# zxhuang1698/ZeroShape

Measured on AMD Instinct MI355X. Metric: sdf_query_points_per_sec_vox128, higher is better.
Workload: dtype f16x3

## Files before the change

### zeroshape_amd/csrc/sdf_decoder_split.hip

```cpp
#include "zs_common.h"
#include <stdlib.h>
#include "sdf_layout.h"
#include "sdf_math.h"
#include "zs_split16.h"
#include "sdf_query.h"
#include "../../include/zeroshape_hip.h"

#include <math.h>
#include <stdint.h>
#include <type_traits>

namespace {

using namespace zs::lay;
using namespace zs::qry;
using zs::dm::gelu_erf;
using zs::dm::softplus100;

typedef float f32x16 __attribute__((ext_vector_type(16)));
typedef float f32x4 __attribute__((ext_vector_type(4)));
typedef float f32x2 __attribute__((ext_vector_type(2)));
typedef unsigned u32x4 __attribute__((ext_vector_type(4)));

constexpr float S_GUARD = 64.0f;
constexpr int KB_U4 = 128;
constexpr int CK = 8;
constexpr int KPW = CK / WAVES;
constexpr int CHUNK_BYTES = CK * KB_U4 * 16;
constexpr int NBUF = 2;
constexpr int KB_TOTAL = G_TOTAL / 2;
constexpr int PRM_WINDOW = 4096;
constexpr int STAGE_FLOATS = NBUF * CHUNK_BYTES / 4;
constexpr int SLAB_TILES = NT - 1;
constexpr int SLAB_U4 = SLAB_TILES * 4 * 64;
constexpr int ZTILES_F4 = NT * 4 * 64;
static_assert(ZSLAB_F4 == 3 * ZTILES_F4, "the workspace slab holds three skip layers' feat partial products");
static_assert(B0_TABLE_FLOATS == PRM_WINDOW, "block0_window_kernel / block0_stream_kernel index an image's table by PRM_WINDOW");
constexpr int LDS_FLOATS = PRM_WINDOW + STAGE_FLOATS + WAVES * SLAB_U4 * 4;
static_assert(LDS_FLOATS * 4 == 160 * 1024, "the kernel owns the whole LDS of a CU");
static_assert(KB_TOTAL % CK == 0 && CK % WAVES == 0 && KPW * 2048 <= 4096, "chunking");
static_assert((RING * GROUP_FLOATS + PARAM_FLOATS) * 4 >= NBUF * CHUNK_BYTES, "prefetch stays inside the program");

constexpr int W_PP = P_PP;
constexpr int W_BLK = P_BLK0;
constexpr int W_IA = P_LNFG;
constexpr int W_IB = P_IMPL_PAIR + P_IMPL_PAIR_STRIDE;
static_assert(P_BLK_STRIDE <= PRM_WINDOW && W_IB - W_IA <= PRM_WINDOW && P_USED - W_IB <= PRM_WINDOW,
              "params windows");

#define DEV __device__ __forceinline__

DEV void pin(u32x4 &a, u32x4 &b) { asm volatile("" : "+v"(a), "+v"(b) : : "memory"); }

using zs::s16::mfma3;
using zs::s16::split2;

struct PT {
    u32x4 v[4];
};
template <typename T>
DEV PT pack_tile(const T &x) {
    PT p;
#pragma unroll
    for (int j = 0; j < 2; j++)
#pragma unroll
        for (int i = 0; i < 4; i++) {
            unsigned h, l;
            split2(x[8 * j + 2 * i], x[8 * j + 2 * i + 1], h, l);
            p.v[2 * j][i] = h;
            p.v[2 * j + 1][i] = l;
        }
    return p;
}

DEV void glds_kblocks(const char *gsrc, unsigned lds_dst) {
#ifdef ZS_EXP_NO_DMA
    if (gsrc != nullptr) return;
#endif
    asm volatile("s_mov_b32 m0, %1\n\ts_nop 0\n\tglobal_load_lds_dwordx4 %0, off"
                 "\n\tglobal_load_lds_dwordx4 %0, off offset:1024"
                 "\n\tglobal_load_lds_dwordx4 %0, off offset:2048"
                 "\n\tglobal_load_lds_dwordx4 %0, off offset:3072"
                 :
                 : "v"(gsrc), "s"(lds_dst)
                 : "memory");
}

struct AStream {
    const u32x4 *buf[NBUF];
    unsigned dst[NBUF];
    u32x4 hi, lo;
    const char *gsrc;

    DEV void init(const char *prog, u32x4 *stage, unsigned stage_addr, int wave, int lane) {
        const char *g = prog + wave * (KPW * KB_U4 * 16) + lane * 16;
        asm volatile("s_waitcnt vmcnt(0) lgkmcnt(0)\n\ts_barrier" ::: "memory");
#pragma unroll
        for (int i = 0; i < NBUF; i++) {
            buf[i] = stage + i * (CK * KB_U4) + lane;
            dst[i] = stage_addr + i * CHUNK_BYTES + wave * (KPW * KB_U4 * 16);
            glds_kblocks(g + i * CHUNK_BYTES, dst[i]);
        }
        gsrc = g + NBUF * CHUNK_BYTES;
        asm volatile("s_waitcnt vmcnt(4)\n\ts_barrier" ::: "memory");
        hi = buf[0][0];
        lo = buf[0][64];
    }
    template <int EXTRA_VM = 0>
    DEV void step(int pos, u32x4 &ahi, u32x4 &alo) {
        ahi = hi;
        alo = lo;
        if (pos == CK - 1) {
            static_assert(EXTRA_VM == 0 || EXTRA_VM == 4, "wait-count variants");
            if (EXTRA_VM == 4)
                asm volatile("s_waitcnt vmcnt(4) lgkmcnt(0)\n\ts_barrier" ::: "memory");
            else
                asm volatile("s_waitcnt vmcnt(0) lgkmcnt(0)\n\ts_barrier" ::: "memory");
            glds_kblocks(gsrc, dst[0]);
            gsrc += CHUNK_BYTES;
            const u32x4 *t = buf[0];
            const unsigned u = dst[0];
            buf[0] = buf[1];
            dst[0] = dst[1];
            buf[1] = t;
            dst[1] = u;
            hi = buf[0][0];
            lo = buf[0][64];
        } else {
#ifndef ZS_EXP_NO_AREAD
            hi = buf[0][(pos + 1) * KB_U4];
            lo = buf[0][(pos + 1) * KB_U4 + 64];
#endif
        }
    }
    DEV void seek(const char *base, int wave, int lane) { gsrc = base + wave * (KPW * KB_U4 * 16) + lane * 16; }
    DEV void drain() { asm volatile("s_waitcnt vmcnt(0) lgkmcnt(0)" ::: "memory"); }
};

struct Slab {
    u32x4 *fl;
    PT t7;
    DEV void store(int tile, const PT &p) {
        if (tile == SLAB_TILES) {
            t7 = p;
        } else {
#pragma unroll
            for (int q = 0; q < 4; q++) fl[(tile * 4 + q) * 64] = p.v[q];
        }
    }
};

DEV f32x16 zero16() {
    f32x16 v;
#pragma unroll
    for (int r = 0; r < 16; r++) v[r] = 0.f;
    return v;
}

struct NoSide {
    DEV void operator()(int, int) const {}
};
template <typename SIDE>
DEV void mfma3_gaps(f32x16 &acc, const u32x4 &ahi, const u32x4 &alo, const u32x4 &bhi, const u32x4 &blo, int kb,
                    SIDE &side) {
    using zs::s16::as_h;
    if (std::is_same<SIDE, NoSide>::value) {
        mfma3(acc, ahi, alo, bhi, blo);
        return;
    }
    acc = __builtin_amdgcn_mfma_f32_32x32x16_f16(as_h(alo), as_h(bhi), acc, 0, 0, 0);
    side(kb, 0);
    acc = __builtin_amdgcn_mfma_f32_32x32x16_f16(as_h(ahi), as_h(blo), acc, 0, 0, 0);
    side(kb, 1);
    acc = __builtin_amdgcn_mfma_f32_32x32x16_f16(as_h(ahi), as_h(bhi), acc, 0, 0, 0);
    side(kb, 2);
}

struct TilePacker {
    PT p;
    float prev;
    DEV void feed(int kb, float v) {
        if (kb & 1) {
            unsigned h, l;
            split2(prev, v, h, l);
            p.v[2 * (kb >> 3)][(kb & 7) >> 1] = h;
            p.v[2 * (kb >> 3) + 1][(kb & 7) >> 1] = l;
        }
        prev = v;
    }
};

struct GeluStager {
    float x, u, q, t, e, p;
    DEV void s0(float v) {
        x = v;
        u = fabsf(v) * 0.70710678118654752440f;
        q = (u * u) * -1.44269504088896340736f;
    }
    DEV void s1() { t = __builtin_amdgcn_rcpf(fmaf(0.3275911f, u, 1.0f)); }
    DEV void s2() {
        e = __builtin_amdgcn_exp2f(q);
        p = fmaf(0.75052702f, t, -1.02753365f);
    }
    DEV void s3() {
        p = fmaf(p, t, 1.00509130f);
        p = fmaf(p, t, -0.20116957f);
        p = fmaf(p, t, 0.18019173f);
        p = p * t;
        u = u * p;
    }
    DEV float s4() const { return fmaf(-u, e, fmaxf(x, 0.0f)); }
    DEV float all(float v) {
        s0(v); s1(); s2(); s3();
        return s4();
    }
    DEV void stage(int st, float v, int idx, TilePacker &pk) {
        if (st == 0) s0(v);
        else if (st == 1) s1();
        else if (st == 2) s2();
        else if (st == 3) s3();
        else if (st == 4) pk.feed(idx, s4());
    }
};
struct SoftplusStager {
    float x, t;
    DEV void s0(float v) {
        x = v;
        t = __builtin_amdgcn_exp2f(fabsf(v) * -144.26950408889634074f);
    }
    DEV void s1() { t = __builtin_amdgcn_logf(1.0f + t); }
    DEV float s2() const { return fmaf(t, 0.0069314718055994530942f, fmaxf(x, 0.0f)); }
};

DEV float kblock_gelu(f32x16 &acc, const u32x4 &ahi, const u32x4 &alo, const u32x4 &bhi, const u32x4 &blo, float x) {
    float u, q, d, t, e, m, p;
    const float c0 = 0.70710678118654752440f, c1 = 0.3275911f, c2 = -1.02753365f;
    asm volatile(
#ifndef ZS_EXP_TWO_TERM
                 "v_mfma_f32_32x32x16_f16 %[acc], %[alo], %[bh], %[acc]\n\t"
#endif
                 "v_mul_f32_e64 %[u], |%[x]|, %[c0]\n\t"
                 "v_mul_f32_e32 %[q], %[u], %[u]\n\t"
                 "v_mul_f32_e32 %[q], 0xbfb8aa3b, %[q]\n\t"
                 "v_fma_f32 %[d], %[u], %[c1], 1.0\n\t"
                 "v_mfma_f32_32x32x16_f16 %[acc], %[ahi], %[bl], %[acc]\n\t"
                 "v_rcp_f32_e32 %[t], %[d]\n\t"
                 "v_exp_f32_e32 %[e], %[q]\n\t"
                 "v_max_f32_e32 %[m], 0, %[x]\n\t"
                 "v_mfma_f32_32x32x16_f16 %[acc], %[ahi], %[bh], %[acc]\n\t"
                 "v_fmamk_f32 %[p], %[t], 0x3f40228a, %[c2]\n\t"
                 "v_fmaak_f32 %[p], %[p], %[t], 0x3f80a6d5\n\t"
                 "v_fmaak_f32 %[p], %[p], %[t], 0xbe4dff65\n\t"
                 "v_fmaak_f32 %[p], %[p], %[t], 0x3e38842e\n\t"
                 "v_mul_f32_e64 %[p], %[t], -%[p]\n\t"
                 "v_mul_f32_e32 %[p], %[u], %[p]\n\t"
                 "v_fmac_f32_e32 %[m], %[p], %[e]"
                 : [acc] "+v"(acc), [u] "=&v"(u), [q] "=&v"(q), [d] "=&v"(d), [t] "=&v"(t), [e] "=&v"(e), [m] "=&v"(m),
                   [p] "=&v"(p)
                 : [alo] "v"(alo), [ahi] "v"(ahi), [bh] "v"(bhi), [bl] "v"(blo), [x] "v"(x), [c0] "s"(c0), [c1] "s"(c1),
                   [c2] "v"(c2));
    return m;
}
DEV float kblock_softplus(f32x16 &acc, const u32x4 &ahi, const u32x4 &alo, const u32x4 &bhi, const u32x4 &blo, float x) {
    float t, m;
    const float c0 = -144.26950408889634074f;
    asm volatile(
#ifndef ZS_EXP_TWO_TERM
                 "v_mfma_f32_32x32x16_f16 %[acc], %[alo], %[bh], %[acc]\n\t"
#endif
                 "v_mul_f32_e64 %[t], |%[x]|, %[c0]\n\t"
                 "v_exp_f32_e32 %[t], %[t]\n\t"
                 "v_mfma_f32_32x32x16_f16 %[acc], %[ahi], %[bl], %[acc]\n\t"
                 "v_max_f32_e32 %[m], 0, %[x]\n\t"
                 "v_add_f32_e32 %[t], 1.0, %[t]\n\t"
                 "v_log_f32_e32 %[t], %[t]\n\t"
                 "v_mfma_f32_32x32x16_f16 %[acc], %[ahi], %[bh], %[acc]\n\t"
                 "s_nop 0\n\t"
                 "v_fmac_f32_e32 %[m], 0x3be32166, %[t]"
                 : [acc] "+v"(acc), [t] "=&v"(t), [m] "=&v"(m)
                 : [alo] "v"(alo), [ahi] "v"(ahi), [bh] "v"(bhi), [bl] "v"(blo), [x] "v"(x), [c0] "s"(c0));
    return m;
}

DEV void mfma_settle(f32x16 &acc) { asm volatile("s_nop 7\n\ts_nop 3" : "+v"(acc)); }

template <int KT, int EXTRA_VM = 0, typename SIDE = NoSide>
DEV void gemm_reg(AStream &s, const PT *X, f32x16 &acc, SIDE side = SIDE()) {
#pragma unroll
    for (int kt = 0; kt < KT; kt++)
#pragma unroll
        for (int j = 0; j < 2; j++) {
            u32x4 ahi, alo;
            s.step((kt * 2 + j) & (CK - 1), ahi, alo);
            pin(ahi, alo);
            mfma3_gaps(acc, ahi, alo, X[kt].v[2 * j], X[kt].v[2 * j + 1], kt * 2 + j, side);
        }
}
template <typename SIDE>
DEV void mfma3_breg(f32x16 &acc, const u32x4 &ahi, const u32x4 &alo, const u32x4 &bhi, const u32x4 &blo, int kb,
                    SIDE &side) {
    asm volatile("s_nop 1\n\tv_mfma_f32_32x32x16_f16 %0, %1, %2, %0" : "+v"(acc) : "v"(alo), "a"(bhi));
    side(kb, 0);
    asm volatile("s_nop 1\n\tv_mfma_f32_32x32x16_f16 %0, %1, %2, %0" : "+v"(acc) : "v"(ahi), "a"(blo));
    side(kb, 1);
    asm volatile("s_nop 1\n\tv_mfma_f32_32x32x16_f16 %0, %1, %2, %0" : "+v"(acc) : "v"(ahi), "a"(bhi));
    side(kb, 2);
}
template <int KT, typename SIDE = NoSide>
DEV void gemm_areg(AStream &s, const PT *X, f32x16 &acc, SIDE side = SIDE()) {
#pragma unroll
    for (int kt = 0; kt < KT; kt++)
#pragma unroll
        for (int j = 0; j < 2; j++) {
            u32x4 ahi, alo;
            s.step((kt * 2 + j) & (CK - 1), ahi, alo);
            pin(ahi, alo);
            mfma3_breg(acc, ahi, alo, X[kt].v[2 * j], X[kt].v[2 * j + 1], kt * 2 + j, side);
        }
}
template <typename SIDE>
DEV void mfma3_cacc(f32x16 &acc, const u32x4 &ahi, const u32x4 &alo, const u32x4 &bhi, const u32x4 &blo, int kb,
                    SIDE &side) {
    asm volatile("s_nop 1\n\tv_mfma_f32_32x32x16_f16 %0, %1, %2, %0" : "+a"(acc) : "v"(alo), "v"(bhi));
    side(kb, 0);
    asm volatile("s_nop 1\n\tv_mfma_f32_32x32x16_f16 %0, %1, %2, %0" : "+a"(acc) : "v"(ahi), "v"(blo));
    side(kb, 1);
    asm volatile("s_nop 1\n\tv_mfma_f32_32x32x16_f16 %0, %1, %2, %0" : "+a"(acc) : "v"(ahi), "v"(bhi));
    side(kb, 2);
}
template <bool YACC = false, typename SIDE = NoSide, int NKB = 2>
DEV void gemm_one(AStream &s, const PT &X, f32x16 &acc, int pos0, int kb0 = 0, SIDE side = SIDE()) {
#pragma unroll
    for (int j = 0; j < NKB; j++) {
        u32x4 ahi, alo;
        s.step((pos0 + j) & (CK - 1), ahi, alo);
        pin(ahi, alo);
        if (YACC)
            mfma3_cacc(acc, ahi, alo, X.v[2 * j], X.v[2 * j + 1], kb0 + j, side);
        else
            mfma3_gaps(acc, ahi, alo, X.v[2 * j], X.v[2 * j + 1], kb0 + j, side);
    }
}
DEV void slab_b(const Slab &sl, int kb, u32x4 &bh, u32x4 &bl) {
    if (kb >= SLAB_TILES * 2) {
        bh = sl.t7.v[(kb & 1) * 2];
        bl = sl.t7.v[(kb & 1) * 2 + 1];
    } else {
        bh = sl.fl[kb * KB_U4];
        bl = sl.fl[kb * KB_U4 + 64];
    }
}
template <typename SIDE = NoSide>
DEV void gemm_lds(AStream &s, const Slab &sl, f32x16 &acc, int pos0 = 0, SIDE side = SIDE()) {
    u32x4 bh, bl;
    slab_b(sl, 0, bh, bl);
#pragma unroll
    for (int kb = 0; kb < NT * 2; kb++) {
        u32x4 ahi, alo;
        s.step((pos0 + kb) & (CK - 1), ahi, alo);
        u32x4 nh = bh, nl = bl;
        if (kb + 1 < NT * 2) slab_b(sl, kb + 1, nh, nl);
        pin(ahi, alo);
        mfma3_gaps(acc, ahi, alo, bh, bl, kb, side);
        bh = nh;
        bl = nl;
    }
}

template <int ACT, typename FIN, typename TAIL>
DEV void gemm_lds_act(AStream &s, const Slab &sl, f32x16 &acc, const f32x16 &cur, FIN fin, TAIL tail) {
    u32x4 bh, bl;
    slab_b(sl, 0, bh, bl);
#pragma unroll
    for (int kb = 0; kb < NT * 2; kb++) {
        u32x4 ahi, alo;
        s.step(kb & (CK - 1), ahi, alo);
        u32x4 nh = bh, nl = bl;
        if (kb + 1 < NT * 2) slab_b(sl, kb + 1, nh, nl);
        const float r = ACT == 0 ? kblock_gelu(acc, ahi, alo, bh, bl, cur[kb]) : kblock_softplus(acc, ahi, alo, bh, bl, cur[kb]);
        bh = nh;
        bl = nl;
        fin(kb, r);
        tail(kb);
    }
}
template <int ACT, typename FIN, typename TAIL>
DEV void gemm_reg_act(AStream &s, const PT *X, f32x16 &acc, const f32x16 &cur, FIN fin, TAIL tail) {
#pragma unroll
    for (int kt = 0; kt < NT; kt++)
#pragma unroll
        for (int j = 0; j < 2; j++) {
            u32x4 ahi, alo;
            const int kb = kt * 2 + j;
            s.step(kb & (CK - 1), ahi, alo);
            const float r = ACT == 0 ? kblock_gelu(acc, ahi, alo, X[kt].v[2 * j], X[kt].v[2 * j + 1], cur[kb])
                                     : kblock_softplus(acc, ahi, alo, X[kt].v[2 * j], X[kt].v[2 * j + 1], cur[kb]);
            fin(kb, r);
            tail(kb);
        }
}

#ifndef ZS_SPLIT_PERMLANE
DEV float half_sum(float v) { return v + __shfl_xor(v, 32, 64); }
DEV float half_max(float v) { return fmaxf(v, __shfl_xor(v, 32, 64)); }
#else
DEV void half_pair(float v, float &lo, float &hi) {
    lo = v;
    hi = v;
    asm volatile("s_nop 4\n\tv_permlane32_swap_b32 %0, %1\n\ts_nop 4" : "+v"(lo), "+v"(hi));
}
DEV float half_sum(float v) {
    float lo, hi;
    half_pair(v, lo, hi);
    return lo + hi;
}
#ifdef ZS_SPLIT_PERMLANE_SUM_ONLY
DEV float half_max(float v) { return fmaxf(v, __shfl_xor(v, 32, 64)); }
#else
DEV float half_max(float v) {
    float lo, hi;
    half_pair(v, lo, hi);
    return fmaxf(lo, hi);
}
#endif
#endif

DEV void rp(const float *prm, int off, int tile, int hi, float *v) {
    const f32x4 *q = reinterpret_cast<const f32x4 *>(prm + off + tile * 32 + hi * 16);
#pragma unroll
    for (int i = 0; i < 4; i++) {
        const f32x4 a = q[i];
        v[4 * i + 0] = a.x; v[4 * i + 1] = a.y; v[4 * i + 2] = a.z; v[4 * i + 3] = a.w;
    }
}
DEV f32x16 rp16(const float *prm, int off, int tile, int hi) {
    float t[16];
    rp(prm, off, tile, hi, t);
    f32x16 v;
#pragma unroll
    for (int r = 0; r < 16; r++) v[r] = t[r];
    return v;
}
constexpr int B0_BPROJ = 0, B0_C = 256, B0_T = 1024;
static_assert(B0_T + HEADS * 3 * 128 == PRM_WINDOW, "the block-0 table is exactly one params window");
constexpr float B0S_LO_SCALE = 64.0f;
constexpr int B0S_KB_HEAD = 34;
static_assert(B0_STREAM_KB == HEADS * B0S_KB_HEAD && B0_STREAM_KB % CK == 0 && B0_STREAM_BYTES == (size_t)B0_STREAM_KB * KB_U4 * 16,
              "the compact stream is whole chunks");
static_assert(B0S_KB_HEAD == 5 + (2 * LT - 1) + 2 * NT && L - 32 * (LT - 1) <= 16, "latent tile 6: rows 16-31 are padding");
DEV void rem2(unsigned h, float a, float b, float &ra, float &rb) {
    asm("v_fma_mix_f32 %0, %1, -1.0, %2 op_sel_hi:[1,0,0]" : "=v"(ra) : "v"(h), "v"(a));
    asm("v_fma_mix_f32 %0, %1, -1.0, %2 op_sel:[1,0,0] op_sel_hi:[1,0,0]" : "=v"(rb) : "v"(h), "v"(b));
}
DEV u32x4 rank5_b(float u0, float u1, float u2, float u3, int hi, bool &bad) {
    using zs::s16::pk_f16;
    const unsigned lim = 0x477fe000u;
    bad = (__builtin_bit_cast(unsigned, u0) & 0x7fffffffu) > lim || (__builtin_bit_cast(unsigned, u1) & 0x7fffffffu) > lim ||
          (__builtin_bit_cast(unsigned, u2) & 0x7fffffffu) > lim || (__builtin_bit_cast(unsigned, u3) & 0x7fffffffu) > lim;
    const unsigned h01 = pk_f16(u0, u1), h23 = pk_f16(u2, u3);
    float r0, r1, r2, r3;
    rem2(h01, u0, u1, r0, r1);
    rem2(h23, u2, u3, r2, r3);
    const float s = B0S_LO_SCALE, is = 1.0f / B0S_LO_SCALE;
    const unsigned l01 = pk_f16(r0 * s, r1 * s), l23 = pk_f16(r2 * s, r3 * s);
    const unsigned d01 = pk_f16((u0 - r0) * is, (u1 - r1) * is), d23 = pk_f16((u2 - r2) * is, (u3 - r3) * is);
    static_assert(B0S_LO_SCALE == 64.0f, "ud4's bit pattern");
    return hi ? u32x4{d01, d23, 0x00003c00u, 0x00002400u} : u32x4{h01, h23, l01, l23};
}
DEV f32x16 mfma_rank5(const u32x4 &a, const u32x4 &ub) {
    return __builtin_amdgcn_mfma_f32_32x32x16_f16(zs::s16::as_h(a), zs::s16::as_h(ub), zero16(), 0, 0, 0);
}

DEV f32x16 xyz_affine(const float *prm, int off, int tile, int hi, float x, float y, float z) {
    const f32x4 *q = reinterpret_cast<const f32x4 *>(prm + off + tile * 128 + hi * 64);
    f32x16 v;
#pragma unroll
    for (int r = 0; r < 16; r++) {
        const f32x4 w = q[r];
        v[r] = fmaf(w.z, z, fmaf(w.y, y, fmaf(w.x, x, w.w)));
    }
    return v;
}

struct XyzInit {
    const f32x4 *q;
    f32x4 w;
    f32x16 v;
    DEV void start(const float *prm, int off, int tile, int hi) {
        q = reinterpret_cast<const f32x4 *>(prm + off + tile * 128 + hi * 64);
        w = q[0];
    }
    DEV void step(int r, float x, float y, float z) {
        v[r] = fmaf(w.z, z, fmaf(w.y, y, fmaf(w.x, x, w.w)));
        if (r + 1 < 16) w = q[r + 1];
    }
};
struct RowInit {
    const f32x4 *q;
    f32x4 w;
    f32x16 v;
    DEV void start(const float *prm, int off, int tile, int hi) {
        q = reinterpret_cast<const f32x4 *>(prm + off + tile * 32 + hi * 16);
        w = q[0];
    }
    DEV void step(int r) {
        if ((r & 3) == 0) {
            v[r] = w.x; v[r + 1] = w.y; v[r + 2] = w.z; v[r + 3] = w.w;
            if (r + 4 < 16) w = q[(r >> 2) + 1];
        }
    }
};

DEV void ln_stats(const f32x16 *x, float &mean, float &rstd) {
    float s = 0.f;
#pragma unroll
    for (int kt = 0; kt < NT; kt++)
#pragma unroll
        for (int r = 0; r < 16; r++) s += x[kt][r];
    s = half_sum(s);
    mean = s * (1.0f / 256.0f);
    float v = 0.f;
#pragma unroll
    for (int kt = 0; kt < NT; kt++)
#pragma unroll
        for (int r = 0; r < 16; r++) {
            const float d = x[kt][r] - mean;
            v = fmaf(d, d, v);
        }
    v = half_sum(v);
    rstd = 1.0f / sqrtf(v * (1.0f / 256.0f) + 1e-6f);
}
DEV void layer_norm_lds(const f32x16 *x, Slab &sl, const float *prm, int g_off, int b_off, int hi) {
    float mean, rstd;
    ln_stats(x, mean, rstd);
#pragma unroll
    for (int kt = 0; kt < NT; kt++) {
        float g[16], b[16], t[16];
        rp(prm, g_off, kt, hi, g);
        rp(prm, b_off, kt, hi, b);
#pragma unroll
        for (int r = 0; r < 16; r++) t[r] = fmaf((x[kt][r] - mean) * rstd, g[r], b[r]);
        sl.store(kt, pack_tile(t));
    }
}

DEV void load_params(float *prm, const float *prog_params, int start, int count) {
    __syncthreads();
    const f32x4 *src = reinterpret_cast<const f32x4 *>(prog_params + start);
    f32x4 *dst = reinterpret_cast<f32x4 *>(prm);
    for (int i = threadIdx.x; i < count / 4; i += WAVES * 64) dst[i] = src[i];
    __syncthreads();
}

template <bool MASK, int NKB = 2>
DEV void softmax_pv(AStream &s, f32x16 &S, f32x16 &o, float &m_run, float &z_run, float c, int hi, int pos0) {
    float mt = -INFINITY;
#pragma unroll
    for (int r = 0; r < 16; r++) {
        if (MASK) {
            const int rw = (r & 3) + 8 * (r >> 2) + 4 * hi;
            S[r] = rw < L - 32 * (LT - 1) ? S[r] : -INFINITY;
        }
        mt = fmaxf(mt, S[r]);
    }
    mt *= c;
    constexpr float LAZY = 8.0f;
    if (__builtin_amdgcn_ballot_w64(mt > m_run + LAZY) != 0) {
        mt = half_max(mt);
        const float m_new = fmaxf(m_run, mt);
        const float alpha = __builtin_amdgcn_exp2f(m_run - m_new);
        z_run *= alpha;
#pragma unroll
        for (int r = 0; r < 16; r++) o[r] *= alpha;
        m_run = m_new;
    }
    float zs_ = 0.f;
#pragma unroll
    for (int r = 0; r < 16; r++) {
        const float p = __builtin_amdgcn_exp2f(fmaf(S[r], c, -m_run));
        S[r] = p;
        zs_ += p;
    }
    z_run += zs_;
    gemm_one<false, NoSide, NKB>(s, pack_tile(S), o, pos0);
}
template <bool MASK>
DEV void attn_tile(AStream &s, const PT &q, f32x16 &o, float &m_run, float &z_run, float c, int hi,
                   int pos0) {
    f32x16 S = zero16();
    gemm_one(s, q, S, pos0);
    softmax_pv<MASK>(s, S, o, m_run, z_run, c, hi, pos0 + 2);
}

DEV void merge_self(f32x16 &o, const f32x16 &v, float m_run, float z_run, float s_self) {
    const float m_new = fmaxf(m_run, s_self);
    const float alpha = __builtin_amdgcn_exp2f(m_run - m_new);
    const float p_self = __builtin_amdgcn_exp2f(s_self - m_new);
    const float z = fmaf(half_sum(z_run), alpha, p_self);
    const float inv = 1.0f / z;
    const float a_i = alpha * inv, p_i = p_self * inv;
#pragma unroll
    for (int r = 0; r < 16; r++) o[r] = fmaf(p_i, v[r], o[r] * a_i);
}

#ifdef ZS_EXP_TIMING
#define ZS_STAMP(i) do { if (dbg) dbg[i] = __builtin_amdgcn_s_memtime(); } while (0)
#else
#define ZS_STAMP(i) do { } while (0)
#endif
DEV float decode_tile(const char *prog, float *prm, u32x4 *stage, unsigned stage_addr, u32x4 *slab,
                      const char *b0s, float px, float py, float pz, int wave, int lane, float &guard,
                      unsigned long long *dbg) {
    const int hi = lane >> 5;
    const float *prog_params = reinterpret_cast<const float *>(prog) + REC_FLOATS;
    AStream s;
    s.init(b0s ? b0s : prog, stage, stage_addr, wave, lane);
    Slab sl;
    sl.fl = slab;
    ZS_STAMP(0);

    load_params(prm, prog_params, W_PP, 1024);
    f32x16 y[NT];
#pragma unroll
    for (int kt = 0; kt < NT; kt++) y[kt] = xyz_affine(prm, 0, kt, hi, px, py, pz);

    ZS_STAMP(1);

    const float scale = 0.17677669529663688110f;

#pragma unroll 1
    for (int blk = 0; blk < BLOCKS; blk++) {
        const bool strm = blk == 0 && b0s != nullptr;
        float rstd0 = 0.f;
        u32x4 ub = {0u, 0u, 0u, 0u};
        bool u_bad = false;
        if (strm) {
            load_params(prm, prog_params, W_BLK, P_BLK_STRIDE);
            float mean;
            ln_stats(y, mean, rstd0);
            ub = rank5_b(px * rstd0, py * rstd0, pz * rstd0, rstd0, hi, u_bad);
        } else {
            load_params(prm, prog_params, W_BLK + blk * P_BLK_STRIDE, P_BLK_STRIDE);
            layer_norm_lds(y, sl, prm, PB_LN1G, PB_LN1B, hi);
        }
        ZS_STAMP(2 + blk * 4);
#pragma unroll
        for (int nt = 0; nt < NT; nt++) y[nt] += rp16(prm, PB_BPROJ, nt, hi);

        auto head = [&](int hd, auto Ptag) {
            constexpr int P = decltype(Ptag)::value;
            f32x16 q = rp16(prm, PB_BQKV, hd * 3 + 0, hi);
            gemm_lds(s, sl, q, P);
            f32x16 k = rp16(prm, PB_BQKV, hd * 3 + 1, hi);
            gemm_lds(s, sl, k, P);
            f32x16 v = rp16(prm, PB_BQKV, hd * 3 + 2, hi);
            gemm_lds(s, sl, v, P);

            const float c = scale * 1.44269504088896340736f;
            float s_self = 0.f;
            float qq = 0.f;
#pragma unroll
            for (int r = 0; r < 16; r++) {
                s_self = fmaf(q[r], k[r], s_self);
                qq = fmaf(q[r], q[r], qq);
            }
            s_self = half_sum(s_self) * c;
            {
                const float km = prog_params[P_KMAX + blk * HEADS + hd] * scale;
                guard = fmaxf(guard, half_sum(qq) * (km * km));
            }
            const PT qp = pack_tile(q);

            float m_run = -INFINITY, z_run = 0.f;
            f32x16 o = zero16();
#pragma unroll
            for (int l2 = 0; l2 < (LT - 1) / 2; l2++) {
                attn_tile<false>(s, qp, o, m_run, z_run, c, hi, P);
                attn_tile<false>(s, qp, o, m_run, z_run, c, hi, (P + 4) & (CK - 1));
            }
            attn_tile<true>(s, qp, o, m_run, z_run, c, hi, P);
            merge_self(o, v, m_run, z_run, s_self);
            const PT op = pack_tile(o);
#pragma unroll
            for (int nt = 0; nt < NT; nt++) gemm_one(s, op, y[nt], (P + 4 + 2 * nt) & (CK - 1));
        };
        auto head_b0s = [&](int hd, auto Ptag) {
            constexpr int P = decltype(Ptag)::value;
            u32x4 a0, a1;
            s.step(P & (CK - 1), a0, a1);
            pin(a0, a1);
            const f32x16 q = mfma_rank5(a0, ub), k = mfma_rank5(a1, ub);
            s.step((P + 1) & (CK - 1), a0, a1);
            pin(a0, a1);
            const f32x16 v = mfma_rank5(a0, ub);
            f32x16 S = mfma_rank5(a1, ub);
            float s_self = 0.f, qq = 0.f;
#pragma unroll
            for (int r = 0; r < 16; r++) {
                s_self = fmaf(q[r], k[r], s_self);
                qq = fmaf(q[r], q[r], qq);
            }
            s_self = half_sum(s_self) * (scale * 1.44269504088896340736f);
            {
                const float km = prog_params[P_KMAX + hd] * scale;
                guard = fmaxf(guard, half_sum(qq) * (km * km));
            }
            float m_run = -INFINITY, z_run = 0.f;
            f32x16 o = zero16();
            softmax_pv<false>(s, S, o, m_run, z_run, 1.0f, hi, P + 2);
#pragma unroll
            for (int i = 0; i < (LT - 1) / 2; i++) {
                s.step((P + 4 + 5 * i) & (CK - 1), a0, a1);
                pin(a0, a1);
                S = mfma_rank5(a0, ub);
                softmax_pv<false>(s, S, o, m_run, z_run, 1.0f, hi, P + 5 + 5 * i);
                S = mfma_rank5(a1, ub);
                if (2 * i + 2 < LT - 1)
                    softmax_pv<false>(s, S, o, m_run, z_run, 1.0f, hi, P + 7 + 5 * i);
                else
                    softmax_pv<true, 1>(s, S, o, m_run, z_run, 1.0f, hi, P + 7 + 5 * i);
            }
            merge_self(o, v, m_run, z_run, s_self);
            const PT op = pack_tile(o);
            if (P == 6 && hd == HEADS - 1) s.seek(prog + HEADS * (G_HEAD / 2) * (KB_U4 * 16), wave, lane);
#pragma unroll
            for (int nt = 0; nt < NT; nt++) gemm_one(s, op, y[nt], (P + 18 + 2 * nt) & (CK - 1));
        };
        static_assert((LT - 1) % 2 == 0 && (3 * NT * 2 + LT * 4 + NT * 2) % CK == 4, "head = 11.5 chunks");
        static_assert(B0S_KB_HEAD % CK == 2 && HEADS % 4 == 0 && (HEADS * (G_HEAD / 2)) % CK == 0,
                      "compact heads start at chunk positions 0, 2, 4, 6; the program resumes on a chunk boundary");
        if (strm) {
#pragma unroll 1
            for (int hd = 0; hd < HEADS; hd += 4) {
                head_b0s(hd, std::integral_constant<int, 0>());
                head_b0s(hd + 1, std::integral_constant<int, 2>());
                head_b0s(hd + 2, std::integral_constant<int, 4>());
                head_b0s(hd + 3, std::integral_constant<int, 6>());
            }
            guard = __builtin_bit_cast(float, u_bad ? 0x7f800000u : __builtin_bit_cast(unsigned, guard));
        } else {
#pragma unroll 1
            for (int hd = 0; hd < HEADS; hd += 2) {
                head(hd, std::integral_constant<int, 0>());
                head(hd + 1, std::integral_constant<int, 4>());
            }
        }

        ZS_STAMP(3 + blk * 4);
        layer_norm_lds(y, sl, prm, PB_LN2G, PB_LN2B, hi);
#pragma unroll
        for (int nt = 0; nt < NT; nt++) y[nt] += rp16(prm, PB_B2, nt, hi);
        ZS_STAMP(4 + blk * 4);
        RowInit bi;
        f32x16 hid = rp16(prm, PB_B1, 0, hi);
        bi.start(prm, PB_B1, 1, hi);
        gemm_lds(s, sl, hid, 0, [&](int kb, int g) {
            if (g == 2 && (kb & 3) == 1) bi.step(kb & ~3);
        });
#pragma unroll 1
        for (int ht = 0; ht < HT - 1; ht++) {
            f32x16 nxt = bi.v;
            bi.start(prm, PB_B1, ht + 2 < HT ? ht + 2 : HT - 1, hi);
            TilePacker e;
            gemm_lds_act<0>(s, sl, nxt, hid, [&](int kb, float r) { e.feed(kb, r); },
                            [&](int kb) { if ((kb & 3) == 1) bi.step(kb & ~3); });
#pragma unroll
            for (int nt = 0; nt < NT; nt++) gemm_one(s, e.p, y[nt], (2 * nt) & (CK - 1));
            hid = nxt;
        }
        {
#pragma unroll
            for (int r = 0; r < 16; r++) hid[r] = gelu_erf(hid[r]);
            const PT hp = pack_tile(hid);
#pragma unroll
            for (int nt = 0; nt < NT; nt++) gemm_one(s, hp, y[nt], (2 * nt) & (CK - 1));
        }
        ZS_STAMP(5 + blk * 4);
    }

    load_params(prm, prog_params, W_IA, W_IB - W_IA);
    float h[NT * 16];
    {
        float mean, rstd;
        ln_stats(y, mean, rstd);
#pragma unroll
        for (int kt = 0; kt < NT; kt++) {
            float g[16], b[16];
            rp(prm, P_LNFG - W_IA, kt, hi, g);
            rp(prm, P_LNFB - W_IA, kt, hi, b);
#pragma unroll
            for (int r = 0; r < 16; r++) h[kt * 16 + r] = fmaf((y[kt][r] - mean) * rstd, g[r], b[r]);
        }
    }
    ZS_STAMP(10);
    PT hp[NT];

#pragma unroll
    for (int kt = 0; kt < NT; kt++) hp[kt] = pack_tile(h + kt * 16);
    {
        f32x16 prev;
        XyzInit ini;
        ini.v = xyz_affine(prm, P_IMPL0 - W_IA, 0, hi, px, py, pz);
#pragma unroll
        for (int nt = 0; nt <= NT; nt++) {
            TilePacker e;
            if (nt < NT) {
                f32x16 acc = ini.v;
                if (nt + 1 < NT) ini.start(prm, P_IMPL0 - W_IA, nt + 1, hi);
                if (nt > 0)
                    gemm_reg_act<1>(s, hp, acc, prev, [&](int kb, float r) { e.feed(kb, r); },
                                    [&](int kb) { if (nt + 1 < NT) ini.step(kb, px, py, pz); });
                else
                    gemm_reg<NT, 0>(s, hp, acc, [&](int kb, int g) { if (g == 2) ini.step(kb, px, py, pz); });
                if (nt > 0) sl.store(nt - 1, e.p);
                prev = acc;
            } else {
                mfma_settle(prev);
#pragma unroll
                for (int kb = 0; kb < 16; kb++) e.feed(kb, softplus100(prev[kb]));
                sl.store(nt - 1, e.p);
            }
        }
    }
    ZS_STAMP(11);
    const float rsqrt2 = 0.70710678118654752440f;
    PT fp[NT];
#pragma unroll
    for (int kt = 0; kt < NT; kt++) {
        float t[16];
#pragma unroll
        for (int r = 0; r < 16; r++) t[r] = h[kt * 16 + r] * rsqrt2;
        fp[kt] = pack_tile(t);
    }
    const float sx = px * rsqrt2, sy = py * rsqrt2, sz = pz * rsqrt2;

    ZS_STAMP(12);
    {
        f32x16 prev;
        RowInit ini;
        ini.v = rp16(prm, P_IMPL1 - W_IA, 0, hi);
#pragma unroll
        for (int nt = 0; nt <= NT; nt++) {
            TilePacker e;
            if (nt < NT) {
                f32x16 acc = ini.v;
                if (nt + 1 < NT) ini.start(prm, P_IMPL1 - W_IA, nt + 1, hi);
                if (nt > 0)
                    gemm_lds_act<1>(s, sl, acc, prev, [&](int kb, float r) { e.feed(kb, r * rsqrt2); },
                                    [&](int kb) { if (nt + 1 < NT) ini.step(kb); });
                else
                    gemm_lds(s, sl, acc, 0, [&](int kb, int g) { if (g == 2) ini.step(kb); });
                if (nt > 0) hp[nt - 1] = e.p;
                prev = acc;
            } else {
                mfma_settle(prev);
#pragma unroll
                for (int kb = 0; kb < 16; kb++) e.feed(kb, softplus100(prev[kb]) * rsqrt2);
                hp[nt - 1] = e.p;
            }
        }
    }
    ZS_STAMP(13);
    float out = 0.f;
#pragma unroll 1
    for (int i = 0; i < 3; i++) {
        if (i == 1) load_params(prm, prog_params, W_IB, P_USED - W_IB);
        const int pp = i == 0 ? P_IMPL_PAIR - W_IA : (i - 1) * P_IMPL_PAIR_STRIDE;
        {
            f32x16 prev;
            XyzInit ini;
            ini.v = xyz_affine(prm, pp, 0, hi, sx, sy, sz);
#pragma unroll
            for (int nt = 0; nt <= NT; nt++) {
                TilePacker e;
                if (nt > 0) mfma_settle(prev);
                if (nt < NT) {
                    f32x16 acc = ini.v;
                    if (nt + 1 < NT) ini.start(prm, pp, nt + 1, hi);
                    if (nt > 0)
                        gemm_reg_act<1>(s, hp, acc, prev, [&](int kb, float r) { e.feed(kb, r); }, [&](int) {});
                    else
                        gemm_reg<NT>(s, hp, acc);
                    gemm_areg<NT>(s, fp, acc, [&](int kb, int g) {
                        if (g == 2 && nt + 1 < NT) ini.step(kb, sx, sy, sz);
                    });
                    if (nt > 0) sl.store(nt - 1, e.p);
                    prev = acc;
                } else {
#pragma unroll
                    for (int kb = 0; kb < 16; kb++) e.feed(kb, softplus100(prev[kb]));
                    sl.store(nt - 1, e.p);
                }
            }
        }
        const float post = i < 2 ? rsqrt2 : 1.0f;
        {
            f32x16 prev;
            RowInit ini, w8;
            const float wsel = i == 2 ? 1.0f : 0.0f;
            ini.v = rp16(prm, pp + 1024, 0, hi);
#pragma unroll
            for (int r = 0; r < 16; r++) w8.v[r] = 0.f;
#pragma unroll
            for (int nt = 0; nt <= NT; nt++) {
                TilePacker e;
                const f32x16 w = w8.v * wsel;
                auto finish = [&](int kb, float v) {
                    const float t = v * post;
                    e.feed(kb, t);
                    out = fmaf(t, w[kb], out);
                };
                if (nt < NT) {
                    f32x16 acc = ini.v;
                    if (nt + 1 < NT) ini.start(prm, pp + 1024, nt + 1, hi);
                    w8.start(prm, P_W8 - W_IB, nt, hi);
                    auto tail = [&](int kb) {
                        if (nt + 1 < NT) ini.step(kb);
                        w8.step(kb);
                    };
                    if (nt > 0)
                        gemm_lds_act<1>(s, sl, acc, prev, [&](int kb, float r) { finish(kb, r); }, tail);
                    else
                        gemm_lds(s, sl, acc, 0, [&](int kb, int g) { if (g == 2) tail(kb); });
                    if (nt > 0) hp[nt - 1] = e.p;
                    prev = acc;
                } else {
                    mfma_settle(prev);
#pragma unroll
                    for (int kb = 0; kb < 16; kb++) finish(kb, softplus100(prev[kb]));
                    hp[nt - 1] = e.p;
                }
            }
        }
    }
    ZS_STAMP(14);
    s.drain();
    out = half_sum(out);
    ZS_STAMP(15);
    return out + prm[P_B8 - W_IB];
}

template <bool GRID>
__global__ __launch_bounds__(WAVES * 64, 1) void sdf_decode_split_kernel(
    const char *__restrict__ programs, size_t program_stride_bytes, int batch,
    const float *__restrict__ points,
    const float *__restrict__ axis,
    int G, long long first_point,
    int m,
    float *__restrict__ out, int apply_sigmoid, f32x4 *__restrict__ workspace,
    int *__restrict__ tile_flags,
    int static_order,
    const char *__restrict__ block0_streams) {
    __shared__ __attribute__((aligned(16))) float lds[LDS_FLOATS];
    float *prm = lds;
    const int lane = threadIdx.x & 63;
    const int wave = __builtin_amdgcn_readfirstlane(threadIdx.x >> 6);
    u32x4 *stage = reinterpret_cast<u32x4 *>(lds + PRM_WINDOW);
    const unsigned stage_addr = __builtin_amdgcn_readfirstlane(
        (unsigned)(uintptr_t)(__attribute__((address_space(3))) float *)(lds + PRM_WINDOW));
    u32x4 *fl = reinterpret_cast<u32x4 *>(lds + PRM_WINDOW + STAGE_FLOATS) + wave * SLAB_U4 + lane;

    const int tiles_per_img = (m + PTS_PER_BLOCK - 1) / PTS_PER_BLOCK;
    const int total = tiles_per_img * batch;
    int *tile_counter = zs::qry::tile_counter(workspace);
    int *tile_slot = tile_counter + 16 + blockIdx.x;
    const int dyn_tiles = total > (int)gridDim.x ? total - (int)gridDim.x : 0;
    for (int tile = blockIdx.x;;) {
      if (tile < total) {
        const int img = tile / tiles_per_img;
        const int t = tile - img * tiles_per_img;
        const char *prog = programs + (size_t)img * program_stride_bytes;

        const int p = t * PTS_PER_BLOCK + wave * PTS_PER_WAVE + (lane & 31);
        const int pc = p < m ? p : m - 1;
        float px, py, pz;
        if (GRID) {
            const long long gp = first_point + pc;
            const long long gg = (long long)G * G;
            const int ix = (int)(gp / gg);
            const int rem = (int)(gp - (long long)ix * gg);
            const int iy = rem / G;
            const int iz = rem - iy * G;
            px = axis[ix];
            py = axis[iy];
            pz = axis[iz];
        } else {
            const float *q = points + ((size_t)img * m + pc) * 3;
            px = q[0];
            py = q[1];
            pz = q[2];
        }
#ifdef ZS_EXP_TIMING
        unsigned long long *dbg = (blockIdx.x == 0 && threadIdx.x == 0 && tile == 0)
            ? timing_stamps(workspace) : nullptr;
#else
        unsigned long long *dbg = nullptr;
#endif
        float guard = 0.f;
        const char *b0s = block0_streams ? block0_streams + (size_t)img * B0_STREAM_BYTES : nullptr;
        float logit = decode_tile(prog, prm, stage, stage_addr, fl, b0s, px, py, pz, wave, lane, guard, dbg);
        if (apply_sigmoid) logit = 1.0f / (1.0f + expf(-logit));
        const unsigned bad = reinterpret_cast<const unsigned *>(prog)[REC_FLOATS + P_FLAG];
        const bool pt_bad = (__builtin_bit_cast(unsigned, px) & 0x7f800000u) == 0x7f800000u ||
                            (__builtin_bit_cast(unsigned, py) & 0x7f800000u) == 0x7f800000u ||
                            (__builtin_bit_cast(unsigned, pz) & 0x7f800000u) == 0x7f800000u;
        if (bad || pt_bad) logit = __builtin_bit_cast(float, 0x7fc00000u);
        if (tile_flags) {
            const bool over = !(__builtin_bit_cast(unsigned, guard) <= __builtin_bit_cast(unsigned, S_GUARD * S_GUARD));
            if (__builtin_amdgcn_ballot_w64(over || bad != 0) != 0 && lane == 0) tile_flags[tile] = 1;
        }
        if (lane < 32 && p < m) out[(size_t)img * m + p] = logit;
      }
        if (static_order) {
            tile += (int)gridDim.x;
            if (tile >= total) break;
            continue;
        }
        if (threadIdx.x == 0) {
            const int d = __hip_atomic_fetch_add(tile_counter, 1, __ATOMIC_RELAXED, __HIP_MEMORY_SCOPE_AGENT);
            if (d == dyn_tiles + (int)gridDim.x - 1)
                __hip_atomic_store(tile_counter, 0, __ATOMIC_RELAXED, __HIP_MEMORY_SCOPE_AGENT);
            __hip_atomic_store(tile_slot, d, __ATOMIC_RELAXED, __HIP_MEMORY_SCOPE_AGENT);
        }
        __syncthreads();
        const int d = __builtin_amdgcn_readfirstlane(__hip_atomic_load(tile_slot, __ATOMIC_RELAXED, __HIP_MEMORY_SCOPE_AGENT));
        if ((unsigned)d >= (unsigned)dyn_tiles) break;
        tile = (int)gridDim.x + d;
    }
}

DEV bool out_of_range(const f32x4 &v) {
    const unsigned lim = 0x477fe000u;
    return (__builtin_bit_cast(unsigned, v.x) & 0x7fffffffu) > lim || (__builtin_bit_cast(unsigned, v.y) & 0x7fffffffu) > lim ||
           (__builtin_bit_cast(unsigned, v.z) & 0x7fffffffu) > lim || (__builtin_bit_cast(unsigned, v.w) & 0x7fffffffu) > lim;
}

__host__ __device__ inline int split_source_kblock(int kb) {
    constexpr int KB_BLOCK = G_BLOCK / 2, KB_ATT = HEADS * G_HEAD / 2;
    static_assert(KB_BLOCK - KB_ATT == HT * 32, "an MLP section is 32 K-blocks per hidden tile");
    constexpr int KB_IMPL0 = BLOCKS * KB_BLOCK, KB_L = NT * NT * 2;
    if (kb >= KB_IMPL0 + G_IMPL / 2) return kb;
    if (kb >= KB_IMPL0) {
        const int p = kb - KB_IMPL0;
        if (p < KB_L) return kb;
        if (p < 2 * KB_L) return KB_IMPL0 + 4 * KB_L + (p - KB_L);
        const int q = p - 2 * KB_L, pair = q / (3 * KB_L), r = q - pair * 3 * KB_L;
        if (r >= 2 * KB_L) return KB_IMPL0 + (5 + 2 * pair + 1) * KB_L + (r - 2 * KB_L);
        const int nt = r / (4 * NT), w = r - nt * 4 * NT;
        return w < 2 * NT ? KB_IMPL0 + (5 + 2 * pair) * KB_L + nt * 2 * NT + w
                          : KB_IMPL0 + (1 + pair) * KB_L + nt * 2 * NT + (w - 2 * NT);
    }
    const int blk = kb / KB_BLOCK, p = kb - blk * KB_BLOCK - KB_ATT;
    if (p < 16) return kb;
    const int q = p - 16, it = q >> 5, r = q & 31;
    int src;
    if (it < HT - 1)
        src = r < 16 ? (it + 1) * 32 + r : it * 32 + r;
    else
        src = it * 32 + 16 + r;
    return blk * KB_BLOCK + KB_ATT + src;
}

__global__ __launch_bounds__(256) void split_program_kernel(const float *__restrict__ src,
                                                            size_t src_stride_floats,
                                                            u32x4 *__restrict__ dst,
                                                            size_t dst_stride_u4) {
    const int img = blockIdx.y;
    const float *s = src + (size_t)img * src_stride_floats;
// ... 313 lines not shown
```

Before: 81.20 million.

## Keep LN2 output in AGPRs instead of LDS slab for MLP GEMMs

The second layer norm output now goes into packed register tiles pinned to AGPRs, where before it was stored to the LDS slab. The MLP up-projection GEMMs then read their B operand straight from those AGPRs through a new gelu kblock variant that takes the B operand in accumulator registers. This is meant to remove LDS stores and reloads on every hidden tile iteration. In exchange it raises accumulator-register pressure, which could cost occupancy or cause spills, and adds an s_nop for the operand hazard.

```diff
diff --git a/zeroshape_amd/csrc/sdf_decoder_split.hip b/zeroshape_amd/csrc/sdf_decoder_split.hip
--- a/zeroshape_amd/csrc/sdf_decoder_split.hip
+++ b/zeroshape_amd/csrc/sdf_decoder_split.hip
@@ -232,35 +232,43 @@
     DEV float s2() const { return fmaf(t, 0.0069314718055994530942f, fmaxf(x, 0.0f)); }
 };
 
-DEV float kblock_gelu(f32x16 &acc, const u32x4 &ahi, const u32x4 &alo, const u32x4 &bhi, const u32x4 &blo, float x) {
-    float u, q, d, t, e, m, p;
-    const float c0 = 0.70710678118654752440f, c1 = 0.3275911f, c2 = -1.02753365f;
-    asm volatile(
 #ifndef ZS_EXP_TWO_TERM
-                 "v_mfma_f32_32x32x16_f16 %[acc], %[alo], %[bh], %[acc]\n\t"
+#define ZS_KBLOCK_MFMA_LO_HI "v_mfma_f32_32x32x16_f16 %[acc], %[alo], %[bh], %[acc]\n\t"
+#else
+#define ZS_KBLOCK_MFMA_LO_HI
 #endif
-                 "v_mul_f32_e64 %[u], |%[x]|, %[c0]\n\t"
-                 "v_mul_f32_e32 %[q], %[u], %[u]\n\t"
-                 "v_mul_f32_e32 %[q], 0xbfb8aa3b, %[q]\n\t"
-                 "v_fma_f32 %[d], %[u], %[c1], 1.0\n\t"
-                 "v_mfma_f32_32x32x16_f16 %[acc], %[ahi], %[bl], %[acc]\n\t"
-                 "v_rcp_f32_e32 %[t], %[d]\n\t"
-                 "v_exp_f32_e32 %[e], %[q]\n\t"
-                 "v_max_f32_e32 %[m], 0, %[x]\n\t"
-                 "v_mfma_f32_32x32x16_f16 %[acc], %[ahi], %[bh], %[acc]\n\t"
-                 "v_fmamk_f32 %[p], %[t], 0x3f40228a, %[c2]\n\t"
-                 "v_fmaak_f32 %[p], %[p], %[t], 0x3f80a6d5\n\t"
-                 "v_fmaak_f32 %[p], %[p], %[t], 0xbe4dff65\n\t"
-                 "v_fmaak_f32 %[p], %[p], %[t], 0x3e38842e\n\t"
-                 "v_mul_f32_e64 %[p], %[t], -%[p]\n\t"
-                 "v_mul_f32_e32 %[p], %[u], %[p]\n\t"
-                 "v_fmac_f32_e32 %[m], %[p], %[e]"
-                 : [acc] "+v"(acc), [u] "=&v"(u), [q] "=&v"(q), [d] "=&v"(d), [t] "=&v"(t), [e] "=&v"(e), [m] "=&v"(m),
-                   [p] "=&v"(p)
-                 : [alo] "v"(alo), [ahi] "v"(ahi), [bh] "v"(bhi), [bl] "v"(blo), [x] "v"(x), [c0] "s"(c0), [c1] "s"(c1),
-                   [c2] "v"(c2));
-    return m;
-}
+#define ZS_KBLOCK_GELU(NAME, BREG, LEAD) \
+DEV float NAME(f32x16 &acc, const u32x4 &ahi, const u32x4 &alo, const u32x4 &bhi, const u32x4 &blo, float x) {             \
+    float u, q, d, t, e, m, p;                                                                                             \
+    const float c0 = 0.70710678118654752440f, c1 = 0.3275911f, c2 = -1.02753365f;                                          \
+    asm volatile(                                                                                                          \
+                 LEAD ZS_KBLOCK_MFMA_LO_HI                                                                                 \
+                 "v_mul_f32_e64 %[u], |%[x]|, %[c0]\n\t"                                                                   \
+                 "v_mul_f32_e32 %[q], %[u], %[u]\n\t"                                                                      \
+                 "v_mul_f32_e32 %[q], 0xbfb8aa3b, %[q]\n\t"                                                                \
+                 "v_fma_f32 %[d], %[u], %[c1], 1.0\n\t"                                                                    \
+                 "v_mfma_f32_32x32x16_f16 %[acc], %[ahi], %[bl], %[acc]\n\t"                                               \
+                 "v_rcp_f32_e32 %[t], %[d]\n\t"                                                                            \
+                 "v_exp_f32_e32 %[e], %[q]\n\t"                                                                            \
+                 "v_max_f32_e32 %[m], 0, %[x]\n\t"                                                                         \
+                 "v_mfma_f32_32x32x16_f16 %[acc], %[ahi], %[bh], %[acc]\n\t"                                               \
+                 "v_fmamk_f32 %[p], %[t], 0x3f40228a, %[c2]\n\t"                                                           \
+                 "v_fmaak_f32 %[p], %[p], %[t], 0x3f80a6d5\n\t"                                                            \
+                 "v_fmaak_f32 %[p], %[p], %[t], 0xbe4dff65\n\t"                                                            \
+                 "v_fmaak_f32 %[p], %[p], %[t], 0x3e38842e\n\t"                                                            \
+                 "v_mul_f32_e64 %[p], %[t], -%[p]\n\t"                                                                     \
+                 "v_mul_f32_e32 %[p], %[u], %[p]\n\t"                                                                      \
+                 "v_fmac_f32_e32 %[m], %[p], %[e]"                                                                         \
+                 : [acc] "+v"(acc), [u] "=&v"(u), [q] "=&v"(q), [d] "=&v"(d), [t] "=&v"(t), [e] "=&v"(e), [m] "=&v"(m),    \
+                   [p] "=&v"(p)                                                                                            \
+                 : [alo] "v"(alo), [ahi] "v"(ahi), [bh] BREG(bhi), [bl] BREG(blo), [x] "v"(x), [c0] "s"(c0), [c1] "s"(c1), \
+                   [c2] "v"(c2));                                                                                          \
+    return m;                                                                                                              \
+}
+ZS_KBLOCK_GELU(kblock_gelu, "v", "")
+ZS_KBLOCK_GELU(kblock_gelu_breg, "a", "s_nop 1\n\t")
+#undef ZS_KBLOCK_GELU
+#undef ZS_KBLOCK_MFMA_LO_HI
 DEV float kblock_softplus(f32x16 &acc, const u32x4 &ahi, const u32x4 &alo, const u32x4 &bhi, const u32x4 &blo, float x) {
     float t, m;
     const float c0 = -144.26950408889634074f;
@@ -399,6 +407,20 @@
             tail(kb);
         }
 }
+template <typename FIN, typename TAIL>
+DEV void gemm_areg_gelu(AStream &s, const PT *X, f32x16 &acc, const f32x16 &cur, FIN fin, TAIL tail) {
+#pragma unroll
+    for (int kt = 0; kt < NT; kt++)
+#pragma unroll
+        for (int j = 0; j < 2; j++) {
+            u32x4 ahi, alo;
+            const int kb = kt * 2 + j;
+            s.step(kb & (CK - 1), ahi, alo);
+            const float r = kblock_gelu_breg(acc, ahi, alo, X[kt].v[2 * j], X[kt].v[2 * j + 1], cur[kb]);
+            fin(kb, r);
+            tail(kb);
+        }
+}
 
 #ifndef ZS_SPLIT_PERMLANE
 DEV float half_sum(float v) { return v + __shfl_xor(v, 32, 64); }
@@ -541,6 +563,26 @@
 #pragma unroll
         for (int r = 0; r < 16; r++) t[r] = fmaf((x[kt][r] - mean) * rstd, g[r], b[r]);
         sl.store(kt, pack_tile(t));
+    }
+}
+#ifndef ZS_SPLIT_LN_SLAB
+constexpr bool LN2_REGS = true;
+#else
+constexpr bool LN2_REGS = false;
+#endif
+DEV void layer_norm_reg(const f32x16 *x, PT *xn, const float *prm, int g_off, int b_off, int hi) {
+    float mean, rstd;
+    ln_stats(x, mean, rstd);
+#pragma unroll
+    for (int kt = 0; kt < NT; kt++) {
+        float g[16], b[16], t[16];
+        rp(prm, g_off, kt, hi, g);
+        rp(prm, b_off, kt, hi, b);
+#pragma unroll
+        for (int r = 0; r < 16; r++) t[r] = fmaf((x[kt][r] - mean) * rstd, g[r], b[r]);
+        xn[kt] = pack_tile(t);
+#pragma unroll
+        for (int q = 0; q < 4; q++) asm volatile("" : "+a"(xn[kt].v[q]));
     }
 }
 
@@ -747,23 +789,37 @@
         }
 
         ZS_STAMP(3 + blk * 4);
-        layer_norm_lds(y, sl, prm, PB_LN2G, PB_LN2B, hi);
+        PT xn[NT];
+        if constexpr (LN2_REGS)
+            layer_norm_reg(y, xn, prm, PB_LN2G, PB_LN2B, hi);
+        else
+            layer_norm_lds(y, sl, prm, PB_LN2G, PB_LN2B, hi);
 #pragma unroll
         for (int nt = 0; nt < NT; nt++) y[nt] += rp16(prm, PB_B2, nt, hi);
         ZS_STAMP(4 + blk * 4);
         RowInit bi;
         f32x16 hid = rp16(prm, PB_B1, 0, hi);
         bi.start(prm, PB_B1, 1, hi);
-        gemm_lds(s, sl, hid, 0, [&](int kb, int g) {
+        auto bias_side = [&](int kb, int g) {
             if (g == 2 && (kb & 3) == 1) bi.step(kb & ~3);
-        });
+        };
+        if constexpr (LN2_REGS) {
+            gemm_areg<NT>(s, xn, hid, bias_side);
+            mfma_settle(hid);
+        } else {
+            gemm_lds(s, sl, hid, 0, bias_side);
+        }
 #pragma unroll 1
         for (int ht = 0; ht < HT - 1; ht++) {
             f32x16 nxt = bi.v;
             bi.start(prm, PB_B1, ht + 2 < HT ? ht + 2 : HT - 1, hi);
             TilePacker e;
-            gemm_lds_act<0>(s, sl, nxt, hid, [&](int kb, float r) { e.feed(kb, r); },
-                            [&](int kb) { if ((kb & 3) == 1) bi.step(kb & ~3); });
+            auto fin = [&](int kb, float r) { e.feed(kb, r); };
+            auto tail = [&](int kb) { if ((kb & 3) == 1) bi.step(kb & ~3); };
+            if constexpr (LN2_REGS)
+                gemm_areg_gelu(s, xn, nxt, hid, fin, tail);
+            else
+                gemm_lds_act<0>(s, sl, nxt, hid, fin, tail);
 #pragma unroll
             for (int nt = 0; nt < NT; nt++) gemm_one(s, e.p, y[nt], (2 * nt) & (CK - 1));
             hid = nxt;
```

New measurement: 82.12 million, median of 6. 1.01x the previous value.
